# ahirner/infur

Hardware: AMD Instinct MI355X
Metric: 1080p frames/sec FCN-ResNet50-12 @1/2/4/8 MI355X; %MFMA roofline (higher is better)
Workload: dtype f32

## Files before the change

### infur_amd/csrc/conv_igemm_kernel.h

```cpp
#pragma once
#include <atomic>
#include <type_traits>

#include "kernels.h"
#include "qepilogue.h"

namespace infur {

#ifdef KTRACE
#ifndef KT_CIN
#define KT_CIN 1024
#define KT_COUT 2048
#endif
static __device__ unsigned long long g_ktrace[8 * 8 * 4];
static inline hipError_t ktrace_read_tu(unsigned long long* out) { return hipMemcpyFromSymbol(out, HIP_SYMBOL(g_ktrace), sizeof(g_ktrace)); }
#endif

typedef float f32x16 __attribute__((ext_vector_type(16)));
typedef _Float16 f16x8 __attribute__((ext_vector_type(8)));
typedef _Float16 f16x4 __attribute__((ext_vector_type(4)));
typedef unsigned int u32x4 __attribute__((ext_vector_type(4)));

constexpr int ROW_BYTES = 128;
constexpr int LDS_ROW = ROW_BYTES + 16;

constexpr unsigned OOB = 0x80000000u;

typedef float f32x4 __attribute__((ext_vector_type(4)));
typedef int i32x4q __attribute__((ext_vector_type(4)));
typedef int i32x16q __attribute__((ext_vector_type(16)));


__device__ __forceinline__ void store_split(char* dst, const u32x4 r, const float scale) {
    const f32x4 x = __builtin_bit_cast(f32x4, r) * scale;
    const f16x4 hi = __builtin_convertvector(x, f16x4);
    const f16x4 lo = __builtin_convertvector(x - __builtin_convertvector(hi, f32x4), f16x4);
    *reinterpret_cast<f16x4*>(dst) = hi;
    *reinterpret_cast<f16x4*>(dst + 64) = lo;
}

typedef int i32x8 __attribute__((ext_vector_type(8)));
__device__ __forceinline__ int pack_fp8x4(const f32x4 v) {
    int w = 0;
    w = __builtin_amdgcn_cvt_pk_bf8_f32(v[0], v[1], w, false);
    w = __builtin_amdgcn_cvt_pk_bf8_f32(v[2], v[3], w, true);
    return w;
}
constexpr float kFp8HiScale = 0.5f, kFp8LoScale = 1024.0f;
constexpr int kFp8CrossScaleA = 127 - 10;
constexpr int kFp8Fmt = 1;
__device__ __forceinline__ void store_split_fp8(char* row, const int chunk, const u32x4 r, const float scale) {
    const f32x4 x = __builtin_bit_cast(f32x4, r) * scale;
    const f16x4 hi = __builtin_convertvector(x, f16x4);
    const f32x4 hf = __builtin_convertvector(hi, f32x4);
    *reinterpret_cast<f16x4*>(row + chunk * 8) = hi;
    *reinterpret_cast<int*>(row + 64 + chunk * 4) = pack_fp8x4(hf * kFp8HiScale);
    *reinterpret_cast<int*>(row + 96 + chunk * 4) = pack_fp8x4((x - hf) * kFp8LoScale);
}

constexpr int lds_row_bytes(int nbuf) { return nbuf >= 4 ? ROW_BYTES : LDS_ROW; }
__host__ __device__ constexpr int lds_swz(int row) { return (row >> 1) & 7; }

constexpr int lds_bytes(int bm, int bn, int wm, int wn, int nbuf) {
    const int operands = (nbuf == 1 ? 1 : 2) * (bm + bn) * lds_row_bytes(nbuf);
    const int staging = wm * wn * 32 * (bn / wn * 4 + 16);
    return operands > staging ? operands : staging;
}

constexpr int min_waves_per_simd(int bm, int bn, int wm, int wn, int nbuf) {
    const int waves = wm * wn;
    const int blocks = 160 * 1024 / lds_bytes(bm, bn, wm, wn, nbuf);
    const int w = blocks * waves / 4;
    return w < 1 ? 1 : (w > 2 ? 2 : w);
}

typedef unsigned u32x4r __attribute__((ext_vector_type(4)));
__device__ __forceinline__ void dma16(const u32x4r rsrc, const unsigned lds, const unsigned voff, const unsigned soff) {
    unsigned keep;
    asm volatile(
        "s_mov_b32 %0, m0\n\t"
        "s_mov_b32 m0, %2\n\t"
        "s_nop 0\n\t"
        "buffer_load_dwordx4 %1, %3, %4 offen lds\n\t"
        "s_mov_b32 m0, %0"
        : "=&s"(keep)
        : "v"(voff), "s"(lds), "s"(rsrc), "s"(soff)
        : "memory");
}
typedef __attribute__((address_space(3))) void lds_void_t;

template <typename T, typename OutT, int BM, int BN, int WM, int WN, int NBUF, bool SPLIT = false, bool G1 = false, bool RESPF = false,
          bool DUAL = false, bool FP8X = false>
__global__ void __launch_bounds__(WM* WN * 64, min_waves_per_simd(BM, BN, WM, WN, NBUF))
    conv_igemm_kernel(const ConvArgs a, const int mtiles, const int ntiles) {
    constexpr bool F32 = std::is_same<T, float>::value && !SPLIT;
    constexpr bool I8 = std::is_same<T, signed char>::value;
    static_assert(!SPLIT || std::is_same<T, float>::value, "SPLIT stages f32 tensors");
    constexpr int ES = sizeof(T);
    constexpr int BK = ROW_BYTES / ES;
    constexpr int NSL = SPLIT ? 2 : 4;
    static_assert(!FP8X || SPLIT, "FP8X is a form of the split mode");
    constexpr int NF = (SPLIT && !FP8X) ? 2 : 1;
    constexpr int NT = WM * WN * 64;
    constexpr int TM = BM / WM / 32;
    constexpr int TN = BN / WN / 32;
    constexpr int A_IT = BM * 8 / NT;
    constexpr int B_IT = BN * 8 / NT;
    static_assert(BM * 8 % NT == 0 && BN * 8 % NT == 0, "tile/threads mismatch");

#ifdef KTRACE
    const unsigned long long kt_start = __builtin_amdgcn_s_memtime();
#endif
    if constexpr (SPLIT) __builtin_amdgcn_s_setreg(1 | (23 << 6) | (0 << 11), 1);
    extern __shared__ __attribute__((aligned(16))) char smem[];
    constexpr bool GLDS = NBUF >= 4;
    static_assert(!GLDS || (!F32 && !SPLIT), "the LDS-DMA form is built for the f16 operands");
    constexpr int LR = lds_row_bytes(NBUF);
    char* As = smem;
    constexpr int NIMG = NBUF == 1 ? 1 : 2;
    char* Bs = smem + NIMG * BM * LR;

    const int nblk = mtiles * ntiles * (a.batch > 1 ? a.batch : 1);
    int tile;
    {
        const int b = blockIdx.x;
        const int xcd = b & 7, loc = b >> 3;
        const int q = nblk >> 3, r = nblk & 7;
        tile = (xcd < r ? xcd * (q + 1) : r * (q + 1) + (xcd - r) * q) + loc;
    }
    const int per_batch = mtiles * ntiles;
    const int bidx = tile / per_batch;
    tile -= bidx * per_batch;
    const int mt = tile / ntiles, nt = tile - mt * ntiles;
    const int m0 = mt * BM, n0 = nt * BN;
    const char* in_base = static_cast<const char*>(a.in) + (size_t)bidx * a.in_bs;
    const char* wt_base = static_cast<const char*>(a.wt) + (size_t)bidx * a.wt_bs;

    const int tid = threadIdx.x;
    const int lane = tid & 63;
    const int wave = tid >> 6;
    const int wm = wave / WN, wn = wave % WN;

    static_assert(!DUAL || (G1 && !RESPF), "DUAL is a form of the 1x1 GEMM addressing");
    constexpr bool CMAJ = std::is_same<T, _Float16>::value && !G1 && !SPLIT;
    const int M = a.OH * a.OW;
    const int Ktot = DUAL ? a.Cin + a.Cin2 : a.KH * a.KW * a.Cin;

    const auto in_rsrc = __builtin_amdgcn_make_buffer_rsrc(
        const_cast<char*>(in_base), 0, (unsigned)((size_t)a.H * a.W * a.Cin * ES), 0x00020000);
    const auto wt_rsrc = __builtin_amdgcn_make_buffer_rsrc(
        const_cast<char*>(wt_base), 0, (unsigned)((size_t)a.Cout * Ktot * ES), 0x00020000);

    int a_iy0[A_IT], a_ix0[A_IT];
    auto st_row = [&](int i, int it) { return GLDS ? 8 * (wave * it + i) + (lane >> 3) : (tid >> 3) + i * (NT / 8); };
    auto st_chunk = [&](int row) { return GLDS ? ((lane & 7) ^ lds_swz(row)) : (tid & 7); };
#pragma unroll
    for (int i = 0; i < A_IT; i++) {
        const int row = st_row(i, A_IT);
        const int c4 = st_chunk(row);
        const int m = m0 + row;
        const int oy = m / a.OW, ox = m - oy * a.OW;
        a_iy0[i] = m < M ? oy * a.stride - a.pad : -0x100000;
        a_ix0[i] = ox * a.stride - a.pad;
        if constexpr (G1)
            a_iy0[i] = m < M ? (int)((unsigned)(oy * a.stride * a.W + ox * a.stride) * (unsigned)(a.Cin * ES) + c4 * 16u) : (int)OOB;
        if constexpr (DUAL)
            a_ix0[i] = m < M ? (int)((unsigned)(oy * a.stride2 * a.W2 + ox * a.stride2) * (unsigned)(a.Cin2 * ES) + c4 * 16u) : (int)OOB;
    }
    const auto in2_rsrc = __builtin_amdgcn_make_buffer_rsrc(const_cast<void*>(DUAL ? a.in2 : a.in), 0,
                                                            DUAL ? (unsigned)((size_t)a.H2 * a.W2 * a.Cin2 * ES) : 0u, 0x00020000);
    unsigned b_off[B_IT];
#pragma unroll
    for (int i = 0; i < B_IT; i++) {
        const int row = st_row(i, B_IT);
        const int n = n0 + row;
        b_off[i] = n < a.Cout ? (unsigned)n * (unsigned)(Ktot * ES) + st_chunk(row) * 16u : OOB;
    }
    u32x4r in_v = {}, in2_v = {}, wt_v = {};
    unsigned lds0 = 0;
    int ld_buf = 0;
    if constexpr (GLDS) {
        auto mk = [](const void* p, unsigned bytes) {
            const unsigned long long v = reinterpret_cast<unsigned long long>(p);
            u32x4r r;
            r.x = __builtin_amdgcn_readfirstlane((unsigned)v);
            r.y = __builtin_amdgcn_readfirstlane((unsigned)(v >> 32) & 0xffffu);
            r.z = __builtin_amdgcn_readfirstlane(bytes);
            r.w = 0x00020000u;
            return r;
        };
        in_v = mk(in_base, (unsigned)((size_t)a.H * a.W * a.Cin * ES));
        wt_v = mk(wt_base, (unsigned)((size_t)a.Cout * Ktot * ES));
        in2_v = mk(DUAL ? a.in2 : a.in, DUAL ? (unsigned)((size_t)a.H2 * a.W2 * a.Cin2 * ES) : 0u);
        lds0 = (unsigned)(size_t)(lds_void_t*)smem;
    }
    auto dst_a = [&](int i) { return __builtin_amdgcn_readfirstlane(lds0 + (unsigned)(ld_buf * BM * LR + (wave * A_IT + i) * 1024)); };
    auto dst_b = [&](int i) { return __builtin_amdgcn_readfirstlane(lds0 + (unsigned)(NIMG * BM * LR + ld_buf * BN * LR + (wave * B_IT + i) * 1024)); };

    f32x16 acc[TM][TN];
#pragma unroll
    for (int i = 0; i < TM; i++)
#pragma unroll
        for (int j = 0; j < TN; j++)
#pragma unroll
            for (int e = 0; e < 16; e++) acc[i][j][e] = 0.0f;

    u32x4 ra[A_IT], rb[B_IT];
    const int cchunks = a.Cin / BK;
    const int ksteps = DUAL ? cchunks + a.Cin2 / BK : a.KH * a.KW * cchunks;
    int ky = 0, kx = 0, cc = 0;

    int kload = 0;
    auto load_a = [&]() {
        if constexpr (G1) {
            if (DUAL && kload >= cchunks) {
                const unsigned so = (unsigned)(kload - cchunks) * (unsigned)ROW_BYTES;
#pragma unroll
                for (int i = 0; i < A_IT; i++) {
                    if constexpr (GLDS)
                        dma16(in2_v, dst_a(i), (unsigned)a_ix0[i], so);
                    else
                        ra[i] = __builtin_amdgcn_raw_buffer_load_b128(in2_rsrc, (unsigned)a_ix0[i], so, 0);
                }
            } else {
                const unsigned so = (unsigned)kload * (unsigned)ROW_BYTES;
#pragma unroll
                for (int i = 0; i < A_IT; i++) {
                    if constexpr (GLDS)
                        dma16(in_v, dst_a(i), (unsigned)a_iy0[i], so);
                    else
                        ra[i] = __builtin_amdgcn_raw_buffer_load_b128(in_rsrc, (unsigned)a_iy0[i], so, 0);
                }
            }
            kload++;
            return;
        }
        const int dy = ky * a.dil, dx = kx * a.dil;
#pragma unroll
        for (int i = 0; i < A_IT; i++) {
            const unsigned coff = (unsigned)(cc * ROW_BYTES + st_chunk(st_row(i, A_IT)) * 16);
            const int iy = a_iy0[i] + dy, ix = a_ix0[i] + dx;
            const bool ok = (unsigned)iy < (unsigned)a.H && (unsigned)ix < (unsigned)a.W;
            const unsigned off = (unsigned)(iy * a.W + ix) * (unsigned)(a.Cin * ES) + coff;
            if constexpr (GLDS)
                dma16(in_v, dst_a(i), ok ? off : OOB, 0u);
            else
                ra[i] = __builtin_amdgcn_raw_buffer_load_b128(in_rsrc, ok ? off : OOB, 0, 0);
        }
        if constexpr (CMAJ) {
            kx += 1;
            const int w1 = kx == a.KW;
            kx = w1 ? 0 : kx;
            ky += w1;
            const int w2 = ky == a.KH;
            ky = w2 ? 0 : ky;
            cc += w2;
        } else {
            cc += 1;
            const int w1 = cc == cchunks;
            cc = w1 ? 0 : cc;
            kx += w1;
            const int w2 = kx == a.KW;
            kx = w2 ? 0 : kx;
            ky += w2;
        }
    };
    auto load_b = [&](int ks) {
        unsigned koff = (unsigned)ks * (unsigned)ROW_BYTES;
        if constexpr (CMAJ) {
            const int taps = a.KH * a.KW, c_ = ks / taps, t_ = ks - c_ * taps;
            koff = (unsigned)(t_ * cchunks + c_) * (unsigned)ROW_BYTES;
        }
#pragma unroll
        for (int i = 0; i < B_IT; i++) {
            if constexpr (GLDS)
                dma16(wt_v, dst_b(i), b_off[i], koff);
            else
                rb[i] = __builtin_amdgcn_raw_buffer_load_b128(wt_rsrc, b_off[i], koff, 0);
        }
    };
    auto load_step = [&](int ks) {
        load_a();
        load_b(ks);
    };
    const int c4 = tid & 7;
    auto store_a = [&](int buf) {
        if constexpr (GLDS) return;
        char* Ab = As + buf * BM * LR;
#pragma unroll
        for (int i = 0; i < A_IT; i++) {
            const int row = (tid >> 3) + i * (NT / 8);
            if constexpr (FP8X)
                store_split_fp8(Ab + row * LR, c4, ra[i], a.a_scale);
            else if constexpr (SPLIT)
                store_split(Ab + row * LR + c4 * 8, ra[i], a.a_scale);
            else
                *reinterpret_cast<u32x4*>(Ab + row * LR + c4 * 16) = ra[i];
        }
    };
    auto store_b = [&](int buf) {
        if constexpr (GLDS) return;
        char* Bb = Bs + buf * BN * LR;
#pragma unroll
        for (int i = 0; i < B_IT; i++) {
            const int row = (tid >> 3) + i * (NT / 8);
            *reinterpret_cast<u32x4*>(Bb + row * LR + c4 * 16) = rb[i];
        }
    };
    auto store_step = [&](int buf) {
        store_a(buf);
        store_b(buf);
    };

    const int a_lds = (wm * TM * 32 + (lane & 31)) * LR + (GLDS ? 0 : (lane >> 5) * 16);
    const int b_lds = (wn * TN * 32 + (lane & 31)) * LR + (GLDS ? 0 : (lane >> 5) * 16);
    const int a_swz = lds_swz(lane & 31), b_swz = a_swz;
    auto read_frags = [&](int buf, int kk, float4 (&fa)[TM * NF], float4 (&fb)[TN * NF]) {
        const char* Ab = As + buf * BM * LR + a_lds + (GLDS ? (((2 * kk + (lane >> 5)) ^ a_swz) * 16) : kk * 32);
        const char* Bb = Bs + buf * BN * LR + b_lds + (GLDS ? (((2 * kk + (lane >> 5)) ^ b_swz) * 16) : kk * 32);
#pragma unroll
        for (int i = 0; i < TM; i++)
#pragma unroll
            for (int p = 0; p < NF; p++) fa[i * NF + p] = *reinterpret_cast<const float4*>(Ab + i * 32 * LR + p * 64);
#pragma unroll
        for (int j = 0; j < TN; j++)
#pragma unroll
            for (int p = 0; p < NF; p++) fb[j * NF + p] = *reinterpret_cast<const float4*>(Bb + j * 32 * LR + p * 64);
    };

    float4 fa[TM * NF], fb[TN * NF], fa_n[TM * NF], fb_n[TN * NF];
    float4 fa8[FP8X ? TM : 1][2], fb8[FP8X ? TN : 1][2];
    const int a_lds8 = (wm * TM * 32 + (lane & 31)) * LR + 64 + (lane >> 5) * 32;
    const int b_lds8 = (wn * TN * 32 + (lane & 31)) * LR + 64 + (lane >> 5) * 32;
    auto read_frags8 = [&](int buf) {
        if constexpr (FP8X) {
            const char* Ab = As + buf * BM * LR + a_lds8;
            const char* Bb = Bs + buf * BN * LR + b_lds8;
#pragma unroll
            for (int i = 0; i < TM; i++) {
                fa8[i][0] = *reinterpret_cast<const float4*>(Ab + i * 32 * LR);
                fa8[i][1] = *reinterpret_cast<const float4*>(Ab + i * 32 * LR + 16);
            }
#pragma unroll
            for (int j = 0; j < TN; j++) {
                fb8[j][0] = *reinterpret_cast<const float4*>(Bb + j * 32 * LR);
                fb8[j][1] = *reinterpret_cast<const float4*>(Bb + j * 32 * LR + 16);
            }
        }
    };

    auto mma_slice = [&](const int kk) {
#pragma unroll
        for (int i = 0; i < TM; i++)
#pragma unroll
            for (int j = 0; j < TN; j++) {
                if constexpr (FP8X) {
                    acc[i][j] = __builtin_amdgcn_mfma_f32_32x32x16_f16(__builtin_bit_cast(f16x8, fb[j]), __builtin_bit_cast(f16x8, fa[i]), acc[i][j], 0, 0, 0);
                    if (kk == 0) {
                        struct F2 { float4 lo, hi; };
                        const i32x8 a8 = __builtin_bit_cast(i32x8, (F2{fa8[i][0], fa8[i][1]}));
                        const i32x8 b8 = __builtin_bit_cast(i32x8, (F2{fb8[j][0], fb8[j][1]}));
                        acc[i][j] = __builtin_amdgcn_mfma_scale_f32_32x32x64_f8f6f4(b8, a8, acc[i][j], kFp8Fmt, kFp8Fmt, 0, kFp8CrossScaleA, 0, 127);
                    }
                } else if constexpr (I8) {
                    const i32x4q ax = __builtin_bit_cast(i32x4q, fa[i]) ^ (int)0x80808080;
                    acc[i][j] = __builtin_bit_cast(f32x16, __builtin_amdgcn_mfma_i32_32x32x32_i8(__builtin_bit_cast(i32x4q, fb[j]), ax,
                                                                                                  __builtin_bit_cast(i32x16q, acc[i][j]), 0, 0, 0));
                } else if constexpr (F32) {
                    acc[i][j] = __builtin_amdgcn_mfma_f32_32x32x2f32(fb[j].x, fa[i].x, acc[i][j], 0, 0, 0);
                    acc[i][j] = __builtin_amdgcn_mfma_f32_32x32x2f32(fb[j].y, fa[i].y, acc[i][j], 0, 0, 0);
                    acc[i][j] = __builtin_amdgcn_mfma_f32_32x32x2f32(fb[j].z, fa[i].z, acc[i][j], 0, 0, 0);
                    acc[i][j] = __builtin_amdgcn_mfma_f32_32x32x2f32(fb[j].w, fa[i].w, acc[i][j], 0, 0, 0);
                } else if constexpr (SPLIT) {
                    const f16x8 ah = __builtin_bit_cast(f16x8, fa[2 * i]), al = __builtin_bit_cast(f16x8, fa[2 * i + 1]);
                    const f16x8 bh = __builtin_bit_cast(f16x8, fb[2 * j]), bl = __builtin_bit_cast(f16x8, fb[2 * j + 1]);
                    acc[i][j] = __builtin_amdgcn_mfma_f32_32x32x16_f16(bh, al, acc[i][j], 0, 0, 0);
                    acc[i][j] = __builtin_amdgcn_mfma_f32_32x32x16_f16(bl, ah, acc[i][j], 0, 0, 0);
                    acc[i][j] = __builtin_amdgcn_mfma_f32_32x32x16_f16(bh, ah, acc[i][j], 0, 0, 0);
                } else {
                    acc[i][j] = __builtin_amdgcn_mfma_f32_32x32x16_f16(__builtin_bit_cast(f16x8, fb[j]),
                                                                     __builtin_bit_cast(f16x8, fa[i]), acc[i][j], 0, 0, 0);
                }
            }
    };

    auto k_step = [&](int ks, auto STORE, auto LOAD, auto NEXT) {
        const int buf = ks & 1;
#pragma unroll
        for (int kk = 0; kk < NSL; kk++) {
            if (kk < NSL - 1)
                read_frags(buf, kk + 1, fa_n, fb_n);
            else if (NEXT)
                read_frags(buf ^ 1, 0, fa_n, fb_n);
            if (kk == 0) read_frags8(buf);
            mma_slice(kk);
            if (kk == 0 && STORE) {
                store_a(buf ^ 1);
                if (LOAD) load_a();
            }
            if (kk == (SPLIT ? 0 : 1) && STORE) {
                store_b(buf ^ 1);
                if (LOAD) load_b(ks + 2);
            }
            if (!F32) {
            } else if (kk <= 1 && STORE) {
#pragma unroll
                for (int g = 0; g < 4; g++) {
                    __builtin_amdgcn_sched_group_barrier(0x8, 1, 0);
                    __builtin_amdgcn_sched_group_barrier(0x100, 1, 0);
                    __builtin_amdgcn_sched_group_barrier(0x2, 4, 0);
                    __builtin_amdgcn_sched_group_barrier(0x8, 1, 0);
                    __builtin_amdgcn_sched_group_barrier(0x200, 1, 0);
                    __builtin_amdgcn_sched_group_barrier(0x2, 4, 0);
                    __builtin_amdgcn_sched_group_barrier(0x8, 1, 0);
                    __builtin_amdgcn_sched_group_barrier(0x20, 1, 0);
                    __builtin_amdgcn_sched_group_barrier(0x2, 4, 0);
                    __builtin_amdgcn_sched_group_barrier(0x8, 1, 0);
                }
            } else {
#pragma unroll
                for (int g = 0; g < 4; g++) {
                    __builtin_amdgcn_sched_group_barrier(0x8, 1, 0);
                    __builtin_amdgcn_sched_group_barrier(0x100, 1, 0);
                    __builtin_amdgcn_sched_group_barrier(0x8, 3, 0);
                }
            }
            if (kk == NSL - 2 && STORE) {
                asm volatile("s_waitcnt lgkmcnt(0)" ::: "memory");
                __builtin_amdgcn_s_barrier();
            }
#pragma unroll
            for (int i = 0; i < TM * NF; i++) fa[i] = fa_n[i];
#pragma unroll
            for (int j = 0; j < TN * NF; j++) fb[j] = fb_n[j];
        }
    };
    constexpr auto Y = std::true_type{};
    constexpr auto N = std::false_type{};

    if constexpr (GLDS) {
        ld_buf = 0;
        load_step(0);
        asm volatile("s_waitcnt vmcnt(0)" ::: "memory");
        __builtin_amdgcn_s_barrier();
    } else {
        load_step(0);
        store_step(0);
        if (ksteps > 1) load_step(1);
        __syncthreads();
    }
#ifdef KTRACE
    const unsigned long long kt_loop = __builtin_amdgcn_s_memtime();
#endif
    constexpr bool Q8 = I8 && std::is_same<OutT, unsigned char>::value;
    constexpr bool H8 = std::is_same<T, _Float16>::value && std::is_same<OutT, _Float16>::value;
    constexpr int CPL = Q8 ? 16 : (H8 ? 8 : 4);
    constexpr int LPR = TN * 32 / CPL;
    constexpr int RPI = 64 / LPR;
    const int e_row = lane / LPR, e_col = lane % LPR;
    const int e_n = n0 + wn * TN * 32 + e_col * CPL;
    const T* res = static_cast<const T*>(a.res);
    using ResV = typename std::conditional<std::is_same<T, float>::value, float4,
                                           typename std::conditional<Q8, u32x4, typename std::conditional<I8, unsigned,
                                           typename std::conditional<H8, f16x8, f16x4>::type>::type>::type>::type;
    ResV rres[RESPF ? TM : 1][RESPF ? 32 / RPI : 1];
    if constexpr (RESPF) {
#pragma unroll
        for (int i = 0; i < TM; i++)
#pragma unroll
            for (int it = 0; it < 32 / RPI; it++) {
                const int m = m0 + wm * TM * 32 + i * 32 + it * RPI + e_row;
                ResV r = {};
                if (m < M && e_n < a.Cout) r = *reinterpret_cast<const ResV*>(res + (size_t)m * a.Cout + e_n);
                rres[i][it] = r;
            }
    }

    if constexpr (NBUF == 3) {
        for (int ks = 0; ks < ksteps; ks++) {
            const int buf = ks & 1;
#pragma unroll
            for (int kk = 0; kk < NSL; kk++) {
                read_frags(buf, kk, fa, fb);
                if (kk == 0) read_frags8(buf);
                mma_slice(kk);
                if (kk == 0 && ks + 1 < ksteps) {
                    store_step(buf ^ 1);
                    if (ks + 2 < ksteps) load_step(ks + 2);
                }
            }
            asm volatile("s_waitcnt lgkmcnt(0)" ::: "memory");
            __builtin_amdgcn_s_barrier();
        }
    } else if constexpr (NBUF >= 4) {
        constexpr bool SPREAD = NBUF == 5;
        for (int ks = 0; ks < ksteps; ks++) {
            const int buf = ks & 1;
            const bool more = ks + 1 < ksteps;
            ld_buf = buf ^ 1;
            if (!SPREAD && more) load_step(ks + 1);
#pragma unroll
            for (int kk = 0; kk < NSL; kk++) {
                read_frags(buf, kk, fa, fb);
                if (SPREAD && more && kk == 0) load_a();
                if (SPREAD && more && kk == 1) load_b(ks + 1);
                mma_slice(kk);
            }
            asm volatile("s_waitcnt vmcnt(0) lgkmcnt(0)" ::: "memory");
            __builtin_amdgcn_s_barrier();
        }
    } else if constexpr (NBUF == 2) {
        read_frags(0, 0, fa, fb);
        int ks = 0;
        for (; ks + 2 < ksteps; ks++) k_step(ks, Y, Y, Y);
        if (ks + 1 < ksteps) k_step(ks++, Y, N, Y);
        k_step(ks, N, N, N);
    } else {
        for (int ks = 0; ks < ksteps; ks++) {
            read_frags(0, 0, fa, fb);
#pragma unroll
            for (int kk = 0; kk < NSL; kk++) {
                if (kk < NSL - 1) read_frags(0, kk + 1, fa_n, fb_n);
                if (kk == 0) read_frags8(0);
                mma_slice(kk);
#pragma unroll
                for (int i = 0; i < TM * NF; i++) fa[i] = fa_n[i];
#pragma unroll
                for (int j = 0; j < TN * NF; j++) fb[j] = fb_n[j];
            }
            if (ks + 1 < ksteps) {
                __syncthreads();
                store_step(0);
                if (ks + 2 < ksteps) load_step(ks + 2);
                __syncthreads();
            }
        }
    }

    OutT* out = reinterpret_cast<OutT*>(static_cast<char*>(a.out) + (size_t)bidx * a.out_bs);
    const float acc_scale = a.acc_scale_b ? a.acc_scale_b[bidx] : a.acc_scale;
    const bool has_bias = a.bias != nullptr;
    const bool vec_ok = I8 || (a.Cout & (CPL - 1)) == 0;
#ifdef KTRACE
    const unsigned long long kt_epi = __builtin_amdgcn_s_memtime();
    struct KtEnd {
        unsigned long long t0, t1, t2; int on, slot;
        __device__ ~KtEnd() {
            asm volatile("s_waitcnt vmcnt(0)" ::: "memory");
            const unsigned long long t3 = __builtin_amdgcn_s_memtime();
            if (on) { g_ktrace[slot * 4 + 0] = t1 - t0; g_ktrace[slot * 4 + 1] = t2 - t1; g_ktrace[slot * 4 + 2] = t3 - t2; }
        }
    } kt_end{kt_start, kt_loop, kt_epi, (a.Cin == KT_CIN && a.Cout == KT_COUT && blockIdx.x < 8 && lane == 0) ? 1 : 0, (int)(blockIdx.x * 8 + wave)};
#endif
    if (vec_ok) {
        constexpr int ROWB = TN * 128 + 16;
        static_assert(NT / 64 * 32 * ROWB <= lds_bytes(BM, BN, WM, WN, NBUF), "epilogue staging exceeds the LDS allocation");
        __syncthreads();
        char* stage = smem + wave * 32 * ROWB;
        const int rrow = e_row, rcol = e_col;
        const int n = e_n;
        const bool n_ok = n < a.Cout;
        float4 bv = make_float4(0.f, 0.f, 0.f, 0.f), bv2 = bv;
        if (has_bias && n_ok) {
            bv = *reinterpret_cast<const float4*>(a.bias + n);
            if constexpr (H8) bv2 = *reinterpret_cast<const float4*>(a.bias + n + 4);
        }
        int qb[CPL];
        float qm[CPL];
#pragma unroll
        for (int t = 0; t < CPL; t++) {
            qb[t] = 0;
            qm[t] = 0.f;
        }
        if constexpr (Q8) {
            if (n_ok) {
#pragma unroll
                for (int t4 = 0; t4 < 4; t4++) {
                    const qi4 b4 = *reinterpret_cast<const qi4*>(a.q_bias + n + 4 * t4);
                    const qf4 m4 = *reinterpret_cast<const qf4*>(a.q_mult + n + 4 * t4);
#pragma unroll
                    for (int t = 0; t < 4; t++) {
                        qb[4 * t4 + t] = b4[t];
                        qm[4 * t4 + t] = m4[t];
                    }
                }
            }
        } else if constexpr (I8) {
#pragma unroll
            for (int t = 0; t < CPL; t++)
                if (n + t < a.Cout) {
                    qb[t] = a.q_bias[n + t];
                    qm[t] = a.q_mult[n + t];
                }
        }
        const float q_yzpf = (float)a.q_yzp, q_lo = -q_yzpf, q_hi = 255.f - q_yzpf;
        const QEpi qe = {q_yzpf, q_lo, q_hi, a.q_ra, a.q_rb, (float)a.q_bzp, (float)a.q_czp};
        float vmax = 0.f;
#pragma unroll
        for (int i = 0; i < TM; i++) {
#pragma unroll
            for (int jj = 0; jj < TN; jj++)
#pragma unroll
                for (int g = 0; g < 4; g++) {
                    float4 v = make_float4(acc[i][jj][4 * g + 0], acc[i][jj][4 * g + 1], acc[i][jj][4 * g + 2], acc[i][jj][4 * g + 3]);
                    if constexpr (SPLIT) {
                        v.x *= acc_scale; v.y *= acc_scale; v.z *= acc_scale; v.w *= acc_scale;
                    }
                    *reinterpret_cast<float4*>(stage + (lane & 31) * ROWB + (jj * 32 + 8 * g + 4 * (lane >> 5)) * 4) = v;
                }
            asm volatile("s_waitcnt lgkmcnt(0)" ::: "memory");
            __builtin_amdgcn_wave_barrier();
            const int mb = m0 + wm * TM * 32 + i * 32;
            ResV rlate[RESPF ? 1 : 32 / RPI];
            if constexpr (!RESPF) {
                if (res) {
#pragma unroll
                    for (int it = 0; it < 32 / RPI; it++) {
                        const int m = mb + it * RPI + rrow;
                        ResV r = {};
                        if (m < M && n_ok) r = *reinterpret_cast<const ResV*>(res + (size_t)m * a.Cout + n);
                        rlate[it] = r;
                    }
                }
            }
#pragma unroll
            for (int it = 0; it < 32 / RPI; it++) {
                const int row = it * RPI + rrow;
                const int m = mb + row;
                float4 v = *reinterpret_cast<const float4*>(stage + row * ROWB + rcol * (CPL * 4));
                if constexpr (Q8) {
                    i32x4q ai[4];
                    ai[0] = __builtin_bit_cast(i32x4q, v);
#pragma unroll
                    for (int t4 = 1; t4 < 4; t4++) ai[t4] = *reinterpret_cast<const i32x4q*>(stage + row * ROWB + rcol * 64 + t4 * 16);
                    if (m < M && n_ok) {
                        u32x4 rv = {0u, 0u, 0u, 0u};
                        const bool has_res = RESPF || res;
                        if (has_res) {
                            if constexpr (RESPF)
                                rv = rres[i][it];
                            else
                                rv = rlate[it];
                        }
                        u32x4 pk;
#pragma unroll
                        for (int t4 = 0; t4 < 4; t4++) {
                            const qi4 a4 = {ai[t4][0] + qb[4 * t4], ai[t4][1] + qb[4 * t4 + 1], ai[t4][2] + qb[4 * t4 + 2], ai[t4][3] + qb[4 * t4 + 3]};
                            const qf4 m4 = {qm[4 * t4], qm[4 * t4 + 1], qm[4 * t4 + 2], qm[4 * t4 + 3]};
                            pk[t4] = has_res ? q_word<true>(a4, m4, rv[t4], qe) : q_word<false>(a4, m4, 0u, qe);
                        }
                        *reinterpret_cast<u32x4*>(out + (size_t)m * a.Cout + n) = pk;
                    }
                } else if constexpr (I8) {
                    if (m < M && n_ok) {
                        const size_t o = (size_t)m * a.Cout + n;
                        const i32x4q ai = __builtin_bit_cast(i32x4q, v);
                        float q[4];
#pragma unroll
                        for (int t = 0; t < 4; t++) q[t] = q_requant_c(ai[t] + qb[t], qm[t], q_lo, q_hi);
                        {
#pragma clang fp contract(off)
                            float4 d;
                            d.x = (q[0] + a.q_dq_off) * a.q_dq; d.y = (q[1] + a.q_dq_off) * a.q_dq;
                            d.z = (q[2] + a.q_dq_off) * a.q_dq; d.w = (q[3] + a.q_dq_off) * a.q_dq;
                            if ((a.Cout & 3) == 0) {
                                *reinterpret_cast<float4*>(out + o) = d;
                            } else {
                                const float dd[4] = {d.x, d.y, d.z, d.w};
#pragma unroll
                                for (int t = 0; t < 4; t++)
                                    if (n + t < a.Cout) out[o + t] = dd[t];
                            }
                        }
                    }
                } else if constexpr (H8) {
                    if (m < M && n_ok) {
                        const float4 v2 = *reinterpret_cast<const float4*>(stage + row * ROWB + rcol * (CPL * 4) + 16);
                        float x[8] = {v.x + bv.x, v.y + bv.y, v.z + bv.z, v.w + bv.w, v2.x + bv2.x, v2.y + bv2.y, v2.z + bv2.z, v2.w + bv2.w};
                        if (RESPF || res) {
                            ResV rv;
                            if constexpr (RESPF)
                                rv = rres[i][it];
                            else
                                rv = rlate[it];
#pragma unroll
                            for (int t = 0; t < 8; t++) x[t] += (float)rv[t];
                        }
                        if (a.relu) {
#pragma unroll
                            for (int t = 0; t < 8; t++) x[t] = fmaxf(x[t], 0.f);
                        }
                        const f16x8 hv = {(_Float16)x[0], (_Float16)x[1], (_Float16)x[2], (_Float16)x[3],
                                          (_Float16)x[4], (_Float16)x[5], (_Float16)x[6], (_Float16)x[7]};
                        *reinterpret_cast<f16x8*>(out + (size_t)m * a.Cout + n) = hv;
                    }
                } else if (m < M && n_ok) {
                    const size_t o = (size_t)m * a.Cout + n;
                    v.x += bv.x; v.y += bv.y; v.z += bv.z; v.w += bv.w;
                    if (RESPF || res) {
                        ResV rv;
                        if constexpr (RESPF)
                            rv = rres[i][it];
                        else
                            rv = rlate[it];
                        if constexpr (std::is_same<T, float>::value) {
                            v.x += rv.x; v.y += rv.y; v.z += rv.z; v.w += rv.w;
                        } else {
                            v.x += (float)rv[0]; v.y += (float)rv[1]; v.z += (float)rv[2]; v.w += (float)rv[3];
                        }
                    }
                    if (a.relu) {
                        v.x = fmaxf(v.x, 0.f); v.y = fmaxf(v.y, 0.f); v.z = fmaxf(v.z, 0.f); v.w = fmaxf(v.w, 0.f);
                    }
                    if constexpr (SPLIT) vmax = fmaxf(vmax, fmaxf(fmaxf(fabsf(v.x), fabsf(v.y)), fmaxf(fabsf(v.z), fabsf(v.w))));
                    if constexpr (std::is_same<OutT, float>::value) {
                        *reinterpret_cast<float4*>(out + o) = v;
                    } else {
                        f16x4 hv = {(_Float16)v.x, (_Float16)v.y, (_Float16)v.z, (_Float16)v.w};
                        *reinterpret_cast<f16x4*>(out + o) = hv;
                    }
                }
            }
            asm volatile("s_waitcnt lgkmcnt(0)" ::: "memory");
            __builtin_amdgcn_wave_barrier();
        }
        if constexpr (SPLIT) {
            if (a.amax) {
#pragma unroll
                for (int o = 32; o > 0; o >>= 1) vmax = fmaxf(vmax, __shfl_xor(vmax, o));
                if (lane == 0 && __float_as_uint(vmax) > *reinterpret_cast<volatile unsigned*>(a.amax)) atomicMax(a.amax, __float_as_uint(vmax));
            }
        }
        return;
    }
#pragma unroll
    for (int i = 0; i < TM; i++) {
        const int m = m0 + wm * TM * 32 + i * 32 + (lane & 31);
        if (m >= M) continue;
#pragma unroll
        for (int j = 0; j < TN; j++) {
#pragma unroll
            for (int g = 0; g < 4; g++) {
                const int n = n0 + wn * TN * 32 + j * 32 + 8 * g + 4 * (lane >> 5);
                if (n >= a.Cout) continue;
                const size_t o = (size_t)m * a.Cout + n;
#pragma unroll
                for (int t = 0; t < 4; t++) {
                    if (n + t >= a.Cout) break;
                    if constexpr (I8) {
                    } else {
                        float x = acc[i][j][4 * g + t];
                        if constexpr (SPLIT) x *= acc_scale;
                        x += has_bias ? a.bias[n + t] : 0.f;
                        if (res) x += (float)res[o + t];
                        if (a.relu) x = fmaxf(x, 0.f);
                        out[o + t] = (OutT)x;
                    }
                }
            }
        }
    }
}

template <typename T, typename OutT, bool SPLIT, bool FP8X, bool G1, bool RESPF, bool DUAL, int BM, int BN, int WM, int WN, int NBUF>
static hipError_t launch_cfg_g(const ConvArgs& a, hipStream_t s) {
    const int M = a.OH * a.OW;
    const int mtiles = (M + BM - 1) / BM;
    const int ntiles = (a.Cout + BN - 1) / BN;
    const size_t lds = (size_t)lds_bytes(BM, BN, WM, WN, NBUF);
    auto k = conv_igemm_kernel<T, OutT, BM, BN, WM, WN, NBUF, SPLIT, G1, RESPF, DUAL, FP8X>;
    static std::atomic<bool> attr_done[64];
    int dev = 0;
    const bool known = hipGetDevice(&dev) == hipSuccess && dev >= 0 && dev < 64;
    if (!known || !attr_done[dev].load(std::memory_order_acquire)) {
        hipError_t e = hipFuncSetAttribute(reinterpret_cast<const void*>(k),
                                           hipFuncAttributeMaxDynamicSharedMemorySize, (int)lds);
        if (e != hipSuccess) return e;
        if (known) attr_done[dev].store(true, std::memory_order_release);
    }
    hipLaunchKernelGGL(k, dim3(mtiles * ntiles * (a.batch > 1 ? a.batch : 1)), dim3(WM * WN * 64), lds, s, a, mtiles, ntiles);
    return hipGetLastError();
}

template <typename T, typename OutT, bool SPLIT, bool FP8X, int BM, int BN, int WM, int WN, int NBUF = 2>
static hipError_t launch_cfg(const ConvArgs& a, hipStream_t s) {
    const bool g1 = a.KH == 1 && a.KW == 1 && a.pad == 0;
    constexpr bool kI8 = std::is_same<T, signed char>::value;
    constexpr bool kSameType = std::is_same<T, OutT>::value || (kI8 && std::is_same<OutT, unsigned char>::value);
    if (kI8 && a.in2) return hipErrorInvalidValue;
    if (kI8 && std::is_same<OutT, unsigned char>::value && (a.Cout & 15)) return hipErrorInvalidValue;
    if (kI8 && std::is_same<OutT, float>::value && a.res) return hipErrorInvalidValue;
    if constexpr (kSameType) {
        if (a.in2) {
            if (!g1 || a.stride != 1 || a.res) return hipErrorInvalidValue;
            return launch_cfg_g<T, OutT, SPLIT, FP8X, true, false, true, BM, BN, WM, WN, NBUF>(a, s);
        }
        constexpr bool kCanPf = (BM / WM) * (BN / WN) <= 64 * 64;
        if constexpr (kCanPf) {
            constexpr int kGroup = (std::is_same<T, _Float16>::value && std::is_same<OutT, _Float16>::value) ? 8 : 4;
            if (a.res && g1 && (a.Cout & (kGroup - 1)) == 0) return launch_cfg_g<T, OutT, SPLIT, FP8X, true, true, false, BM, BN, WM, WN, NBUF>(a, s);
        }
    } else if (a.in2) {
        return hipErrorInvalidValue;
    }
    if (g1) return launch_cfg_g<T, OutT, SPLIT, FP8X, true, false, false, BM, BN, WM, WN, NBUF>(a, s);
    return launch_cfg_g<T, OutT, SPLIT, FP8X, false, false, false, BM, BN, WM, WN, NBUF>(a, s);
}

template <typename T, typename OutT, bool SPLIT, bool FP8X, int I>
static hipError_t launch_form(const ConvArgs& a, hipStream_t s) {
    constexpr ConvForm f = kConvForms[I];
    constexpr ConvMode kMode = std::is_same<T, signed char>::value ? kModeI8 : std::is_same<T, _Float16>::value ? kModeF16
                               : !SPLIT ? kModeF32 : FP8X ? kModeSplitFp8 : kModeSplit;
    if constexpr ((f.modes & mode_bit(kMode)) != 0 && f.family == kFamTiled) {
        return launch_cfg<T, OutT, SPLIT, FP8X, f.bm, f.bn, f.wm, f.wn, f.stage>(a, s);
    } else if constexpr ((f.modes & mode_bit(kMode)) != 0 && !std::is_same<OutT, float>::value) {
        if constexpr (f.family == kFamHalo) {
            return kMode == kModeI8 ? launch_conv3x3_halo_q(a, f.bn, s) : launch_conv3x3_halo(a, f.bn, s);
        } else if constexpr (f.family == kFamHalo4) {
            return launch_conv3x3_halo4(a, s);
        } else if constexpr (kMode == kModeI8) {
            const int nsplit = f.family == kFamAreg ? 1 : conv1x1_q8_nsplit(a);
            if (conv1x1_q8_valid(a, kMode, 0) && (f.family == kFamAreg || nsplit > 1)) return launch_conv1x1_q8(a, nsplit, s);
        } else {
            if (conv1x1_areg_valid(a, kMode, 0)) return launch_conv1x1_areg(a, s);
        }
    }
    return hipErrorInvalidValue;
}

template <typename T, typename OutT, bool SPLIT = false, bool FP8X = false>
static hipError_t launch_t(const ConvArgs& a, int cfg, hipStream_t s) {
    constexpr size_t ES = sizeof(T);
    if (a.Cin % (int)(ROW_BYTES / ES) != 0 || (a.in2 && a.Cin2 % (int)(ROW_BYTES / ES) != 0)) return hipErrorInvalidValue;
    if ((size_t)a.H * a.W * a.Cin * ES >= 0x80000000ull || (size_t)a.Cout * a.KH * a.KW * a.Cin * ES >= 0x80000000ull)
        return hipErrorInvalidValue;
    return conv_form_visit<0, kNumConvCfgs>(cfg, hipErrorInvalidValue, [&](auto row) { return launch_form<T, OutT, SPLIT, FP8X, decltype(row)::value>(a, s); });
}

}
```

Before: 104.4.

## Issue both prologue k-step loads before waiting and prefetch bias during final step

For f32 double-buffered tiles, the prologue now computes weight offsets and issues the weight loads first, then pixel coordinates and A loads, then the second k-step's loads, all before waiting only for the first step's data. This overlaps address setup and accumulator zeroing with global-memory latency. It also loads the bias vector before the last k-step so the epilogue does not stall on it. The cost is extra registers for the second staging set (ra0/rb0), which may lower occupancy.

```diff
diff --git a/infur_amd/csrc/conv_igemm_kernel.h b/infur_amd/csrc/conv_igemm_kernel.h
--- a/infur_amd/csrc/conv_igemm_kernel.h
+++ b/infur_amd/csrc/conv_igemm_kernel.h
@@ -14,6 +14,9 @@
 #endif
 static __device__ unsigned long long g_ktrace[8 * 8 * 4];
 static inline hipError_t ktrace_read_tu(unsigned long long* out) { return hipMemcpyFromSymbol(out, HIP_SYMBOL(g_ktrace), sizeof(g_ktrace)); }
+#define KT_STAMP(v) v = __builtin_amdgcn_s_memtime()
+#else
+#define KT_STAMP(v) ((void)0)
 #endif
 
 typedef float f32x16 __attribute__((ext_vector_type(16)));
@@ -72,6 +75,12 @@
     const int blocks = 160 * 1024 / lds_bytes(bm, bn, wm, wn, nbuf);
     const int w = blocks * waves / 4;
     return w < 1 ? 1 : (w > 2 ? 2 : w);
+}
+
+constexpr bool pro2_fits(int bm, int bn, int nbuf, bool g1) {
+    if (nbuf == 1) return false;
+    if (bm == 256 && bn == 32 && !g1) return false;
+    return true;
 }
 
 typedef unsigned u32x4r __attribute__((ext_vector_type(4)));
@@ -110,6 +119,7 @@
 
 #ifdef KTRACE
     const unsigned long long kt_start = __builtin_amdgcn_s_memtime();
+    unsigned long long kt_w0 = 0, kt_w1 = 0;
 #endif
     if constexpr (SPLIT) __builtin_amdgcn_s_setreg(1 | (23 << 6) | (0 << 11), 1);
     extern __shared__ __attribute__((aligned(16))) char smem[];
@@ -154,27 +164,51 @@
     int a_iy0[A_IT], a_ix0[A_IT];
     auto st_row = [&](int i, int it) { return GLDS ? 8 * (wave * it + i) + (lane >> 3) : (tid >> 3) + i * (NT / 8); };
     auto st_chunk = [&](int row) { return GLDS ? ((lane & 7) ^ lds_swz(row)) : (tid & 7); };
-#pragma unroll
-    for (int i = 0; i < A_IT; i++) {
-        const int row = st_row(i, A_IT);
-        const int c4 = st_chunk(row);
-        const int m = m0 + row;
-        const int oy = m / a.OW, ox = m - oy * a.OW;
-        a_iy0[i] = m < M ? oy * a.stride - a.pad : -0x100000;
-        a_ix0[i] = ox * a.stride - a.pad;
-        if constexpr (G1)
-            a_iy0[i] = m < M ? (int)((unsigned)(oy * a.stride * a.W + ox * a.stride) * (unsigned)(a.Cin * ES) + c4 * 16u) : (int)OOB;
-        if constexpr (DUAL)
-            a_ix0[i] = m < M ? (int)((unsigned)(oy * a.stride2 * a.W2 + ox * a.stride2) * (unsigned)(a.Cin2 * ES) + c4 * 16u) : (int)OOB;
-    }
+    constexpr bool PRO2 = F32 && !GLDS && pro2_fits(BM, BN, NBUF, G1);
     const auto in2_rsrc = __builtin_amdgcn_make_buffer_rsrc(const_cast<void*>(DUAL ? a.in2 : a.in), 0,
                                                             DUAL ? (unsigned)((size_t)a.H2 * a.W2 * a.Cin2 * ES) : 0u, 0x00020000);
     unsigned b_off[B_IT];
-#pragma unroll
-    for (int i = 0; i < B_IT; i++) {
-        const int row = st_row(i, B_IT);
-        const int n = n0 + row;
-        b_off[i] = n < a.Cout ? (unsigned)n * (unsigned)(Ktot * ES) + st_chunk(row) * 16u : OOB;
+    auto pixel_coords = [&] {
+#pragma unroll
+        for (int i = 0; i < A_IT; i++) {
+            const int row = st_row(i, A_IT);
+            const int c4 = st_chunk(row);
+            const int m = m0 + row;
+            const int oy = m / a.OW, ox = m - oy * a.OW;
+            a_iy0[i] = m < M ? oy * a.stride - a.pad : -0x100000;
+            a_ix0[i] = ox * a.stride - a.pad;
+            if constexpr (G1) a_iy0[i] = m < M ? (int)((unsigned)(oy * a.stride * a.W + ox * a.stride) * (unsigned)(a.Cin * ES) + c4 * 16u) : (int)OOB;
+            if constexpr (DUAL) a_ix0[i] = m < M ? (int)((unsigned)(oy * a.stride2 * a.W2 + ox * a.stride2) * (unsigned)(a.Cin2 * ES) + c4 * 16u) : (int)OOB;
+        }
+    };
+    auto weight_rows = [&] {
+#pragma unroll
+        for (int i = 0; i < B_IT; i++) {
+            const int row = st_row(i, B_IT);
+            const int n = n0 + row;
+            b_off[i] = n < a.Cout ? (unsigned)n * (unsigned)(Ktot * ES) + st_chunk(row) * 16u : OOB;
+        }
+    };
+    if constexpr (!PRO2) {
+#pragma unroll
+        for (int i = 0; i < A_IT; i++) {
+            const int row = st_row(i, A_IT);
+            const int c4 = st_chunk(row);
+            const int m = m0 + row;
+            const int oy = m / a.OW, ox = m - oy * a.OW;
+            a_iy0[i] = m < M ? oy * a.stride - a.pad : -0x100000;
+            a_ix0[i] = ox * a.stride - a.pad;
+            if constexpr (G1)
+                a_iy0[i] = m < M ? (int)((unsigned)(oy * a.stride * a.W + ox * a.stride) * (unsigned)(a.Cin * ES) + c4 * 16u) : (int)OOB;
+            if constexpr (DUAL)
+                a_ix0[i] = m < M ? (int)((unsigned)(oy * a.stride2 * a.W2 + ox * a.stride2) * (unsigned)(a.Cin2 * ES) + c4 * 16u) : (int)OOB;
+        }
+#pragma unroll
+        for (int i = 0; i < B_IT; i++) {
+            const int row = st_row(i, B_IT);
+            const int n = n0 + row;
+            b_off[i] = n < a.Cout ? (unsigned)n * (unsigned)(Ktot * ES) + st_chunk(row) * 16u : OOB;
+        }
     }
     u32x4r in_v = {}, in2_v = {}, wt_v = {};
     unsigned lds0 = 0;
@@ -198,20 +232,24 @@
     auto dst_b = [&](int i) { return __builtin_amdgcn_readfirstlane(lds0 + (unsigned)(NIMG * BM * LR + ld_buf * BN * LR + (wave * B_IT + i) * 1024)); };
 
     f32x16 acc[TM][TN];
-#pragma unroll
-    for (int i = 0; i < TM; i++)
-#pragma unroll
-        for (int j = 0; j < TN; j++)
-#pragma unroll
-            for (int e = 0; e < 16; e++) acc[i][j][e] = 0.0f;
+    auto zero_acc = [&] {
+#pragma unroll
+        for (int i = 0; i < TM; i++)
+#pragma unroll
+            for (int j = 0; j < TN; j++)
+#pragma unroll
+                for (int e = 0; e < 16; e++) acc[i][j][e] = 0.0f;
+    };
+    if constexpr (!PRO2) zero_acc();
 
     u32x4 ra[A_IT], rb[B_IT];
+    u32x4 ra0[PRO2 ? A_IT : 1], rb0[PRO2 ? B_IT : 1];
     const int cchunks = a.Cin / BK;
     const int ksteps = DUAL ? cchunks + a.Cin2 / BK : a.KH * a.KW * cchunks;
     int ky = 0, kx = 0, cc = 0;
 
     int kload = 0;
-    auto load_a = [&]() {
+    auto load_a_to = [&](auto& dst, const bool en = true) {
         if constexpr (G1) {
             if (DUAL && kload >= cchunks) {
                 const unsigned so = (unsigned)(kload - cchunks) * (unsigned)ROW_BYTES;
@@ -220,7 +258,7 @@
                     if constexpr (GLDS)
                         dma16(in2_v, dst_a(i), (unsigned)a_ix0[i], so);
                     else
-                        ra[i] = __builtin_amdgcn_raw_buffer_load_b128(in2_rsrc, (unsigned)a_ix0[i], so, 0);
+                        dst[i] = __builtin_amdgcn_raw_buffer_load_b128(in2_rsrc, en ? (unsigned)a_ix0[i] : OOB, so, 0);
                 }
             } else {
                 const unsigned so = (unsigned)kload * (unsigned)ROW_BYTES;
@@ -229,7 +267,7 @@
                     if constexpr (GLDS)
                         dma16(in_v, dst_a(i), (unsigned)a_iy0[i], so);
                     else
-                        ra[i] = __builtin_amdgcn_raw_buffer_load_b128(in_rsrc, (unsigned)a_iy0[i], so, 0);
+                        dst[i] = __builtin_amdgcn_raw_buffer_load_b128(in_rsrc, en ? (unsigned)a_iy0[i] : OOB, so, 0);
                 }
             }
             kload++;
@@ -245,7 +283,7 @@
             if constexpr (GLDS)
                 dma16(in_v, dst_a(i), ok ? off : OOB, 0u);
             else
-                ra[i] = __builtin_amdgcn_raw_buffer_load_b128(in_rsrc, ok ? off : OOB, 0, 0);
+                dst[i] = __builtin_amdgcn_raw_buffer_load_b128(in_rsrc, ok && en ? off : OOB, 0, 0);
         }
         if constexpr (CMAJ) {
             kx += 1;
@@ -265,7 +303,8 @@
             ky += w2;
         }
     };
-    auto load_b = [&](int ks) {
+    auto load_a = [&] { load_a_to(ra); };
+    auto load_b_to = [&](int ks, auto& dst, const bool en = true) {
         unsigned koff = (unsigned)ks * (unsigned)ROW_BYTES;
         if constexpr (CMAJ) {
             const int taps = a.KH * a.KW, c_ = ks / taps, t_ = ks - c_ * taps;
@@ -276,37 +315,40 @@
             if constexpr (GLDS)
                 dma16(wt_v, dst_b(i), b_off[i], koff);
             else
-                rb[i] = __builtin_amdgcn_raw_buffer_load_b128(wt_rsrc, b_off[i], koff, 0);
-        }
-    };
+                dst[i] = __builtin_amdgcn_raw_buffer_load_b128(wt_rsrc, en ? b_off[i] : OOB, koff, 0);
+        }
+    };
+    auto load_b = [&](int ks) { load_b_to(ks, rb); };
     auto load_step = [&](int ks) {
         load_a();
         load_b(ks);
     };
     const int c4 = tid & 7;
-    auto store_a = [&](int buf) {
+    auto store_a_from = [&](int buf, const auto& src) {
         if constexpr (GLDS) return;
         char* Ab = As + buf * BM * LR;
 #pragma unroll
         for (int i = 0; i < A_IT; i++) {
             const int row = (tid >> 3) + i * (NT / 8);
             if constexpr (FP8X)
-                store_split_fp8(Ab + row * LR, c4, ra[i], a.a_scale);
+                store_split_fp8(Ab + row * LR, c4, src[i], a.a_scale);
             else if constexpr (SPLIT)
-                store_split(Ab + row * LR + c4 * 8, ra[i], a.a_scale);
+                store_split(Ab + row * LR + c4 * 8, src[i], a.a_scale);
             else
-                *reinterpret_cast<u32x4*>(Ab + row * LR + c4 * 16) = ra[i];
-        }
-    };
-    auto store_b = [&](int buf) {
+                *reinterpret_cast<u32x4*>(Ab + row * LR + c4 * 16) = src[i];
+        }
+    };
+    auto store_a = [&](int buf) { store_a_from(buf, ra); };
+    auto store_b_from = [&](int buf, const auto& src) {
         if constexpr (GLDS) return;
         char* Bb = Bs + buf * BN * LR;
 #pragma unroll
         for (int i = 0; i < B_IT; i++) {
             const int row = (tid >> 3) + i * (NT / 8);
-            *reinterpret_cast<u32x4*>(Bb + row * LR + c4 * 16) = rb[i];
-        }
-    };
+            *reinterpret_cast<u32x4*>(Bb + row * LR + c4 * 16) = src[i];
+        }
+    };
+    auto store_b = [&](int buf) { store_b_from(buf, rb); };
     auto store_step = [&](int buf) {
         store_a(buf);
         store_b(buf);
@@ -441,10 +483,32 @@
     if constexpr (GLDS) {
         ld_buf = 0;
         load_step(0);
+        KT_STAMP(kt_w0);
         asm volatile("s_waitcnt vmcnt(0)" ::: "memory");
+        KT_STAMP(kt_w1);
         __builtin_amdgcn_s_barrier();
+    } else if constexpr (PRO2) {
+        const bool more = ksteps > 1;
+        weight_rows();
+        load_b_to(0, rb0);
+        pixel_coords();
+        load_a_to(ra0);
+        load_a_to(ra, more);
+        load_b_to(1, rb, more);
+        zero_acc();
+        KT_STAMP(kt_w0);
+        asm volatile("s_waitcnt vmcnt(%0)" ::"n"(A_IT + B_IT) : "memory");
+        KT_STAMP(kt_w1);
+        store_a_from(0, ra0);
+        store_b_from(0, rb0);
+        __syncthreads();
     } else {
         load_step(0);
+#ifdef KTRACE
+        KT_STAMP(kt_w0);
+        asm volatile("s_waitcnt vmcnt(0)" ::: "memory");
+        KT_STAMP(kt_w1);
+#endif
         store_step(0);
         if (ksteps > 1) load_step(1);
         __syncthreads();
@@ -464,6 +528,8 @@
                                            typename std::conditional<Q8, u32x4, typename std::conditional<I8, unsigned,
                                            typename std::conditional<H8, f16x8, f16x4>::type>::type>::type>::type;
     ResV rres[RESPF ? TM : 1][RESPF ? 32 / RPI : 1];
+    constexpr bool BIASPF = F32 && NBUF == 2;
+    float4 bv_pf = make_float4(0.f, 0.f, 0.f, 0.f);
     if constexpr (RESPF) {
 #pragma unroll
         for (int i = 0; i < TM; i++)
@@ -514,6 +580,9 @@
         int ks = 0;
         for (; ks + 2 < ksteps; ks++) k_step(ks, Y, Y, Y);
         if (ks + 1 < ksteps) k_step(ks++, Y, N, Y);
+        if constexpr (BIASPF) {
+            if (a.bias != nullptr && (a.Cout & (CPL - 1)) == 0 && e_n < a.Cout) bv_pf = *reinterpret_cast<const float4*>(a.bias + e_n);
+        }
         k_step(ks, N, N, N);
     } else {
         for (int ks = 0; ks < ksteps; ks++) {
@@ -544,13 +613,13 @@
 #ifdef KTRACE
     const unsigned long long kt_epi = __builtin_amdgcn_s_memtime();
     struct KtEnd {
-        unsigned long long t0, t1, t2; int on, slot;
+        unsigned long long t0, t1, t2, tw; int on, slot;
         __device__ ~KtEnd() {
             asm volatile("s_waitcnt vmcnt(0)" ::: "memory");
             const unsigned long long t3 = __builtin_amdgcn_s_memtime();
-            if (on) { g_ktrace[slot * 4 + 0] = t1 - t0; g_ktrace[slot * 4 + 1] = t2 - t1; g_ktrace[slot * 4 + 2] = t3 - t2; }
-        }
-    } kt_end{kt_start, kt_loop, kt_epi, (a.Cin == KT_CIN && a.Cout == KT_COUT && blockIdx.x < 8 && lane == 0) ? 1 : 0, (int)(blockIdx.x * 8 + wave)};
+            if (on) { g_ktrace[slot * 4 + 0] = t1 - t0; g_ktrace[slot * 4 + 1] = t2 - t1; g_ktrace[slot * 4 + 2] = t3 - t2; g_ktrace[slot * 4 + 3] = tw; }
+        }
+    } kt_end{kt_start, kt_loop, kt_epi, kt_w1 - kt_w0, (a.Cin == KT_CIN && a.Cout == KT_COUT && blockIdx.x < 8 && lane == 0) ? 1 : 0, (int)(blockIdx.x * 8 + wave)};
 #endif
     if (vec_ok) {
         constexpr int ROWB = TN * 128 + 16;
@@ -560,8 +629,8 @@
         const int rrow = e_row, rcol = e_col;
         const int n = e_n;
         const bool n_ok = n < a.Cout;
-        float4 bv = make_float4(0.f, 0.f, 0.f, 0.f), bv2 = bv;
-        if (has_bias && n_ok) {
+        float4 bv = bv_pf, bv2 = make_float4(0.f, 0.f, 0.f, 0.f);
+        if (!BIASPF && has_bias && n_ok) {
             bv = *reinterpret_cast<const float4*>(a.bias + n);
             if constexpr (H8) bv2 = *reinterpret_cast<const float4*>(a.bias + n + 4);
         }
```

Result: no change. 104.1 (-0.3%).
